# musaru/Fall_Multimodal

Measured on AMD Instinct MI355X. Metric: clips/sec (fwd+bwd) 3-stream Fall3, B=256, 1/2/4/8 GPUs; top-1 acc parity, higher is better.
Workload: dtype bf16x3; 1 GPU; fall3_3stream_coco_mmpose_V18_S6_B256_per_gpu; global_batch=256, seq_len=30, parallelism=dp1, joints=18, imu_axes=6, classes=11, hip_graph=False, ranks=1

## Files before the change

### fall_multimodal_amd/_lib.py

```python
from __future__ import annotations

import ctypes
import os

import torch

HERE = os.path.dirname(os.path.abspath(__file__))
LIB_PATH = os.environ.get("F3_LIB") or os.path.join(HERE, "libfall3.so")

EXPORTS = (
    "f3_net_create", "f3_net_destroy", "f3_net_num_entries", "f3_net_entry", "f3_net_param_count",
    "f3_net_buffer_count", "f3_net_counter_count", "f3_net_workspace_bytes", "f3_net_forward",
    "f3_net_loss", "f3_net_backward", "f3_rmsprop_step", "f3_conv_forward", "f3_status_string",
    "f3_net_debug_tensor", "f3_conv_backward_data", "f3_conv_backward_weight", "f3_conv_wgrad_packed", "f3_split_x3cat",
    "f3_conv_forward_x3cat", "f3_conv_backward_data_x3cat", "f3_conv_backward_weight_x3cat", "f3_conv_step_x3cat", "f3_graph_mix_forward",
    "f3_graph_mix_backward", "f3_graph_mix_forward_ex", "f3_graph_mix_backward_ex", "f3_gcn_dgrad_mix_x3",
    "f3_net_backward_phase",
    "f3_net_grad_split", "f3_net_wait_phase1", "f3_net_backward_rmsprop", "f3_net_fused_rmsprop", "f3_net_precision", "f3_net_status",
    "f3_targcn_create", "f3_targcn_destroy", "f3_targcn_num_entries", "f3_targcn_entry", "f3_targcn_param_count",
    "f3_targcn_buffer_count", "f3_targcn_workspace_bytes", "f3_targcn_forward", "f3_targcn_backward", "f3_targcn_stage_times", "f3_targcn_status", "f3_net_sensor_times", "f3_soft_ce",
    "f3_sktr_create", "f3_sktr_destroy", "f3_sktr_num_entries", "f3_sktr_entry", "f3_sktr_param_count",
    "f3_sktr_buffer_count", "f3_sktr_counter_count", "f3_sktr_workspace_bytes", "f3_sktr_forward", "f3_sktr_backward",
    "f3_musa_create", "f3_musa_destroy", "f3_musa_num_entries", "f3_musa_entry", "f3_musa_param_count",
    "f3_musa_buffer_count", "f3_musa_counter_count", "f3_musa_workspace_bytes", "f3_musa_forward", "f3_musa_backward",
    "f3_musa_guards",
    "f3_dwconv_t_forward", "f3_pointwise_conv", "f3_rgb_scratch_floats", "f3_rgb_forward", "f3_rgb_backward",
    "f3_optim_scalars_bytes", "f3_optim_step", "f3_optim_step_ranges", "f3_net_backward_optim", "f3_net_entry_nograd",
)

F3_OK, F3_EINVAL, F3_EBATCH, F3_EHIP, F3_ESTATE, F3_EDEVICE = 0, 1001, 1002, 1003, 1004, 1005
ENTRY_PARAM, ENTRY_BUFFER, ENTRY_COUNTER = 0, 1, 2
OPT_RMSPROP, OPT_SGD, OPT_ADAM, OPT_ADAMW = 0, 1, 2, 3
OPT_MAX_SKIP = 4


class F3OptimConfig(ctypes.Structure):
    _fields_ = ([("kind", ctypes.c_int), ("nesterov", ctypes.c_int)]
                + [(n, ctypes.c_double) for n in ("lr", "alpha", "eps", "momentum", "beta1", "beta2", "weight_decay",
                                                  "max_norm", "grad_scale")]
                + [("nskip", ctypes.c_int), ("skip_lo", ctypes.c_int64 * OPT_MAX_SKIP),
                   ("skip_len", ctypes.c_int64 * OPT_MAX_SKIP)])


class F3TargcnConfig(ctypes.Structure):
    _fields_ = [(n, ctypes.c_int) for n in ("num_node", "num_class", "precision")]


class F3MusaConfig(ctypes.Structure):
    _fields_ = [(n, ctypes.c_int) for n in ("num_point", "frames", "num_class", "precision")]


class F3SktrConfig(ctypes.Structure):
    _fields_ = [(n, ctypes.c_int) for n in ("num_joint", "frames", "persons", "num_class", "precision")]


class F3Config(ctypes.Structure):
    _fields_ = [(n, ctypes.c_int) for n in (
        "model", "num_node", "num_partition", "num_class", "in_channels", "sensor", "sensor_dim",
        "sensor_classes", "softmax_output", "naming", "frames", "sensor_frames", "precision")]


_lib = None


def lib():
    global _lib
    if _lib is not None:
        return _lib
    if not os.path.exists(LIB_PATH):
        raise RuntimeError(f"fall3: {LIB_PATH} is not built (run `make` or __graft_entry__.build())")
    L = ctypes.CDLL(LIB_PATH)
    P, I, I64, F = ctypes.c_void_p, ctypes.c_int, ctypes.c_int64, ctypes.c_float
    sig = {
        "f3_net_create": (I, [ctypes.POINTER(F3Config), ctypes.POINTER(P)]),
        "f3_net_destroy": (None, [P]),
        "f3_net_num_entries": (I, [P]),
        "f3_net_entry": (I, [P, I, ctypes.POINTER(ctypes.c_char_p), ctypes.POINTER(I), ctypes.POINTER(I),
                             ctypes.POINTER(I64), ctypes.POINTER(I64)]),
        "f3_net_param_count": (I64, [P]),
        "f3_net_buffer_count": (I64, [P]),
        "f3_net_counter_count": (I64, [P]),
        "f3_net_workspace_bytes": (I64, [P, I]),
        "f3_net_forward": (I, [P, I, I, P, P, P, P, P, P, P, P]),
        "f3_net_loss": (I, [P, I, P, P, P, P, P]),
        "f3_net_backward": (I, [P, I, P, P, P, P, P]),
        "f3_net_backward_phase": (I, [P, I, P, P, P, P, I, P]),
        "f3_net_grad_split": (I64, [P]),
        "f3_net_wait_phase1": (I, [P, P]),
        "f3_net_backward_rmsprop": (I, [P, I, P, P, P, P, P, F, F, F, P]),
        "f3_net_fused_rmsprop": (I, [P]),
        "f3_net_precision": (I, [P]),
        "f3_net_status": (I, [P, I]),
        "f3_rmsprop_step": (I, [P, P, P, I64, F, F, F, F, P]),
        "f3_optim_scalars_bytes": (I64, []),
        "f3_optim_step": (I, [ctypes.POINTER(F3OptimConfig), P, P, P, P, I64, P, P]),
        "f3_optim_step_ranges": (I, [ctypes.POINTER(F3OptimConfig), P, P, P, P, I, ctypes.POINTER(I64),
                                     ctypes.POINTER(I64), P, P]),
        "f3_net_backward_optim": (I, [P, I, P, P, P, P, P, P, P, ctypes.POINTER(F3OptimConfig), P]),
        "f3_net_entry_nograd": (I, [P, I]),
        "f3_conv_forward": (I, [P, P, P, P, P, I, I, I, I, I, I, I, I, I, P]),
        "f3_status_string": (ctypes.c_char_p, [I]),
        "f3_net_debug_tensor": (P, [P, I, P, I, I, ctypes.c_char_p]),
        "f3_conv_backward_data": (I, [P, P, P, P, I, I, I, I, I, I, I, I, I, P]),
        "f3_conv_backward_weight": (I, [P, P, P, P, I, I, I, I, I, I, I, I, I, P]),
        "f3_conv_wgrad_packed": (I, [P, P, P, ctypes.c_longlong, I, I, I, I, I, I, I, I, P]),
        "f3_split_x3cat": (I, [P, P, ctypes.c_int64, I, P]),
        "f3_conv_forward_x3cat": (I, [P, P, P, P, P, I, I, I, I, I, I, I, I, P]),
        "f3_conv_backward_data_x3cat": (I, [P, P, P, P, I, I, I, I, I, I, I, I, P]),
        "f3_conv_backward_weight_x3cat": (I, [P, P, P, P, I, I, I, I, I, I, I, I, P]),
        "f3_conv_step_x3cat": (I, [I, P, P, P, P, P, P, P, P, P, P, F, P, P, I, I, I, I, I, P]),
        "f3_graph_mix_forward": (I, [P, P, P, I, I, I, I, P]),
        "f3_graph_mix_backward": (I, [P, P, P, P, P, I, I, I, I, P]),
        "f3_graph_mix_forward_ex": (I, [P, P, P, I, I, I, I, I, P]),
        "f3_graph_mix_backward_ex": (I, [P, P, P, P, P, I, I, I, I, I, P]),
        "f3_gcn_dgrad_mix_x3": (I, [P, P, P, P, P, P, P, I, I, I, I, I, I, I, P]),
        "f3_targcn_create": (I, [ctypes.POINTER(F3TargcnConfig), ctypes.POINTER(P)]),
        "f3_targcn_destroy": (None, [P]),
        "f3_targcn_num_entries": (I, [P]),
        "f3_targcn_entry": (I, [P, I, ctypes.POINTER(ctypes.c_char_p), ctypes.POINTER(I), ctypes.POINTER(I),
                                ctypes.POINTER(I64), ctypes.POINTER(I64)]),
        "f3_targcn_param_count": (I64, [P]),
        "f3_targcn_buffer_count": (I64, [P]),
        "f3_targcn_workspace_bytes": (I64, [P, I]),
        "f3_targcn_stage_times": (I, [P, I, P]),
        "f3_targcn_status": (I, [P, I]),
        "f3_net_sensor_times": (I, [P, I, P]),
        "f3_targcn_forward": (I, [P, I, P, P, P, P, P, P]),
        "f3_targcn_backward": (I, [P, I, P, P, P, P, P, P]),
        "f3_soft_ce": (I, [P, P, I, I, P, P, P]),
        "f3_sktr_create": (I, [ctypes.POINTER(F3SktrConfig), ctypes.POINTER(P)]),
        "f3_sktr_destroy": (None, [P]),
        "f3_sktr_num_entries": (I, [P]),
        "f3_sktr_entry": (I, [P, I, ctypes.POINTER(ctypes.c_char_p), ctypes.POINTER(I), ctypes.POINTER(I),
                              ctypes.POINTER(I64), ctypes.POINTER(I64)]),
        "f3_sktr_param_count": (I64, [P]),
        "f3_sktr_buffer_count": (I64, [P]),
        "f3_sktr_counter_count": (I64, [P]),
        "f3_sktr_workspace_bytes": (I64, [P, I]),
        "f3_sktr_forward": (I, [P, I, I, P, P, P, P, P, P, P, ctypes.c_uint, F, P]),
        "f3_sktr_backward": (I, [P, I, P, P, P, P, P, P]),
        "f3_musa_create": (I, [ctypes.POINTER(F3MusaConfig), ctypes.POINTER(P)]),
        "f3_musa_destroy": (None, [P]),
        "f3_musa_num_entries": (I, [P]),
        "f3_musa_entry": (I, [P, I, ctypes.POINTER(ctypes.c_char_p), ctypes.POINTER(I), ctypes.POINTER(I),
                              ctypes.POINTER(I64), ctypes.POINTER(I64)]),
        "f3_musa_param_count": (I64, [P]),
        "f3_musa_buffer_count": (I64, [P]),
        "f3_musa_counter_count": (I64, [P]),
        "f3_musa_workspace_bytes": (I64, [P, I]),
        "f3_musa_guards": (I, [P, I, ctypes.POINTER(I64), I]),
        "f3_musa_forward": (I, [P, I, I, P, P, P, P, P, P, ctypes.c_uint, I, P]),
        "f3_musa_backward": (I, [P, I, P, P, P, P, P, P]),
        "f3_dwconv_t_forward": (I, [P, P, P, P, P, I, I, I, I, I, I, I, P]),
        "f3_pointwise_conv": (I, [P, P, P, P, I, P, P, I, I, I, I, I, I, I, I, I, P]),
        "f3_rgb_scratch_floats": (ctypes.c_longlong, [I, I]),
        "f3_rgb_forward": (I, [P, P, P, P, I, I, P]),
        "f3_rgb_backward": (I, [P, P, P, P, P, P, P, ctypes.c_longlong, I, I, P]),
    }
    for name, (res, args) in sig.items():
        fn = getattr(L, name)
        fn.restype = res
        fn.argtypes = args
    _lib = L
    return L


def check(status: int, what: str):
    if status == F3_OK:
# ... 19 lines not shown
```

### fall_multimodal_amd/csrc/layers.h

```cpp
#pragma once
#include "common.h"

namespace f3 {

enum : int { PREP_MUL = 0, PREP_PACK_CONV, PREP_PACK_CONV_T, PREP_PACK_GCN, PREP_PACK_GCN_T, PREP_GCN_BIAS, PREP_COPY,
              PREP_UNPACK_CONV };

struct PrepJob {
  int type, n;
  float* dst;
  const float* s0;
  const float* s1;
  const float* s2;
  int d0, d1, d2;
  int bf16;
};

struct DataBnArgs {
  int N, T, V, C, motion;
  const float* skel;
  float* out;
  int act16;
  BnRef bn;
  double* st_sum;
  double* st_sq;
  const float* dout;
  float* dgamma;
  float* dbeta;
  float* part;
};

struct MixArgs {
  int K, V, Cin, frames;
  const float* A;
  const float* x;
  int x16;
  float* z;
  float* dx;
  float* dA;
  int accumulate;
  float* part;
  unsigned short* zb;
  const unsigned short* dzb;
  int no_colsum;
  int x3;
  unsigned short* z3;
};
constexpr int kMixParts = 1024;

struct GcnDgradMixArgs {
  int frames, K, V, Cin, C;
  const unsigned short* dg;
  const unsigned short* w;
  const float* A;
  const float* x;
  float* dx;
  float* dA;
  int accumulate;
  float* part;
  int no_colsum;
  int max_workgroups;
};

struct Gcn0Args {
  int frames, K, V, Ci;
  const float* A;
  const unsigned short* x;
  const unsigned short* w;
  const float* beff;
  unsigned short* z;
  unsigned short* g;
  double* st_sum;
  double* st_sq;
  const unsigned short* dg;
  float* dx;
  int accumulate;
  float* part_dA;
  float* part_dW;
  int f32;
};

struct GcnBiasBwdArgs {
  int K, V, C;
  const float* Aeff;
  const float* A;
  const float* G;
  const float* bias;
  float* db;
  const float* dAeff;
  float* dE;
};

enum : int { RES_NONE = 0, RES_ID = 1, RES_CONV = 2 };

constexpr int kCaMaxRowsPerThread = 4;

struct BlockArgs {
  int N, TV, C, chunks, res_kind;
  int act16;
  float inv_tv;
  BnRef bn2, bnr;
  const float* h;
  const float* r;
  const float* x;
  const float* att;
  float* out;
  float* pool;
  unsigned short* outb;
  const float* dout;
  const float* dout_nc;
  float* P1;
  float* P2;
  float* Q2;
  double* bnr_bsum;
// ... 61 lines not shown
  const float* Q2;
  double* bnr_bsum;
  double* bnr_bsq;
  float* dq2;
  float* dbn;
  float* dq1;
  float* e;
  double* bn2_bsum;
  double* bn2_bsq;
  float* g_bnca_gamma;
  float* g_bnca_beta;
  float* g_b1;
  float* g_W1;
  float* g_W2;
  float* g_b2;
  float* wpart;
  const float* bpart;
  int bchunks;
};


struct BnRunJob {
  const double* sum;
  const double* sumsq;
  double count;
  int C;
  float* rmean;
  float* rvar;
  long long* nbt;
};

constexpr int kMaxPrepJobs = 56;
struct PrepTable {
  int n;
  PrepJob jobs[kMaxPrepJobs];
};
constexpr int kMaxBnJobs = 56;
struct BnRunTable {
  int n;
  BnRunJob jobs[kMaxBnJobs];
};

}

int f3_prep(const f3::PrepTable& t, hipStream_t s);
int f3_databn_fwd(const f3::DataBnArgs* a, hipStream_t s);
int f3_databn_bwd(const f3::DataBnArgs* a, hipStream_t s);
int f3_mix_fwd(const f3::MixArgs* a, hipStream_t s);
int f3_mix_bwd(const f3::MixArgs* a, hipStream_t s);
int f3_mix_bwd_parts(const f3::MixArgs* a);
bool f3_gcn_dgrad_mix_ok(int K, int V, int Cin, int C);
int f3_gcn_dgrad_mix(const f3::GcnDgradMixArgs* a, hipStream_t s);
int f3_gcn_dgrad_mix_parts(const f3::GcnDgradMixArgs* a);
bool f3_mix_lds_ok(int K, int V, int Cin);
bool f3_mix_x3_ok(int K, int V, int Cin);
int f3_split_x3(const float* x, unsigned short* out, long long rows, int C, hipStream_t s);
int f3_gcn_bias_bwd(const f3::GcnBiasBwdArgs* a, hipStream_t s);
bool f3_gcn0_ok(int K, int V, int Ci, int C);
int f3_gcn0_fwd(const f3::Gcn0Args* a, hipStream_t s);
int f3_gcn0_bwd(const f3::Gcn0Args* a, hipStream_t s);
int f3_gcn0_bwd_parts(const f3::Gcn0Args* a);
int f3_databn_bwd2(const f3::DataBnArgs* a, hipStream_t s);
int f3_block_out(f3::BlockArgs a, hipStream_t s);
int f3_block_bwd_reduce(f3::BlockArgs a, hipStream_t s);
int f3_block_bwd_apply(f3::BlockArgs a, hipStream_t s);
int f3_bn_bwd_apply(f3::BnBwdArgs a, hipStream_t s);
int f3_bn_bwd_parts(int N, int TV, int V);
int f3_block_chunks(int TV);
int f3_bnrelu_bf16(const f3::BnReluArgs* a, hipStream_t s);
constexpr int kColsumJobs = 10;
struct ColsumJob {
  const float* part;
  float* out;
  long long ld;
  int rows, cols;
};
int f3_colsum_multi(const ColsumJob* jobs, int n, hipStream_t s);
int f3_colsum(const float* part, int rows, int cols, float* out, hipStream_t s);
int f3_colsum_ld(const float* part, int rows, long long ld, int cols, float* out, hipStream_t s);
int f3_ca_fwd(const f3::CaArgs* a, hipStream_t s);
int f3_ca_bwd(const f3::CaArgs* a, hipStream_t s);
int f3_ca_bwd_weights(const f3::CaArgs* a, hipStream_t s, ColsumJob* defer = nullptr, int* ndefer = nullptr);
bool f3_ca_x_ok(int N, int C, int TV);
int f3_bn_running(const f3::BnRunTable& t, hipStream_t s);
```

### fall_multimodal_amd/csrc/net.cpp

```cpp
#include <hip/hip_runtime.h>

#include <algorithm>
#include <cstdio>
#include <functional>
#include <cstdlib>
#include <cstring>
#include <string>
#include <vector>

#include "common.h"
#include "status_ring.h"
#include "kernels.h"
#include "layers.h"
#include "sensor.h"
#include "fall3.h"

using namespace f3;

namespace {

struct Entry {
  std::string name;
  int kind;
  std::vector<int64_t> shape;
// ... 439 lines not shown
  float* G;
  float* opt_p = nullptr;
  float* opt_sq = nullptr;
  float lr = 0.f, alpha = 0.f, eps = 0.f;
  const OptLaunch* opt_gen = nullptr;
  const float* p(int i) const { return P + net.entries[i].offset; }
  float* g(int i) const { return G + net.entries[i].offset; }
  float* b(int i) const { return B + net.entries[i].offset; }
  long long* c(int i) const { return reinterpret_cast<long long*>(C + net.entries[i].offset); }
  BnRef ref(const BnIdx& bi, const BnWs& w, float count, int eval) const {
    BnRef r;
    r.sum = w.fsum;
    r.sumsq = w.fsq;
    r.gamma = p(bi.w);
    r.beta = p(bi.b);
    r.rmean = B ? b(bi.rm) : nullptr;
    r.rvar = B ? b(bi.rv) : nullptr;
    r.count = count;
    r.eval = eval;
    return r;
  }
};


ConvGeom geom(int M, int Nc, int Kc, int KT, int S, int P, int tr, int T_out, int T_in, int V, int lda, int ldo) {
  ConvGeom g;
  g.M = M; g.Nc = Nc; g.Kc = Kc; g.KT = KT; g.S = S; g.P = P; g.transposed = tr;
  g.T_out = T_out; g.T_in = T_in; g.V = V; g.lda = lda; g.ldo = ldo;
  return g;
}

void add_job(PrepTable& t, int type, int n, float* dst, const float* s0, const float* s1, const float* s2, int d0,
             int d1, int d2, int bf16 = 0) {
  PrepJob& j = t.jobs[t.n++];
  j.type = type; j.n = n; j.dst = dst; j.s0 = s0; j.s1 = s1; j.s2 = s2; j.d0 = d0; j.d1 = d1; j.d2 = d2;
  j.bf16 = bf16;
}

inline const unsigned short* bf(const float* p, int on) { return on ? reinterpret_cast<const unsigned short*>(p) : nullptr; }
inline int is_x3(const f3_net& n) { return n.cfg.precision == F3_PRECISION_BF16X3; }
inline int side_pct(bool split, int l) { return split && l >= 2 ? 75 : 0; }
constexpr int x3code() { return 4; }
inline int x3mul(int code) { return code == 4 ? 2 : 1; }
inline void x3_gemm(ConvGemmArgs& a, int C) {
  a.x3n = 1;
  a.g.lda = 2 * C;
}

inline bool gcn_dgrad_fused() {
  static const bool on = !getenv("F3_GCN_DGRAD_FUSED") || atoi(getenv("F3_GCN_DGRAD_FUSED")) != 0;
  return on;
}

inline int wcode(const f3_net& n) { return n.cfg.precision == F3_PRECISION_BF16 ? 1 : is_x3(n) ? 2 : 0; }
inline unsigned short* bfa(float* p, int on) { return on ? reinterpret_cast<unsigned short*>(p) : nullptr; }

void add_bnrun(BnRunTable& t, const Ptrs& q, const BnIdx& bi, const double* sum, const double* sq, double count) {
  BnRunJob& j = t.jobs[t.n++];
  j.sum = sum; j.sumsq = sq; j.count = count; j.C = bi.C;
  j.rmean = q.b(bi.rm); j.rvar = q.b(bi.rv); j.nbt = q.c(bi.nbt);
}

int stream_forward_layer(const f3_net& net, int si, int N, int train, const Ptrs& q, Ws& w, BnRunTable& run,
                         hipStream_t s, int l);

int stream_forward(const f3_net& net, int si, int N, int train, const Ptrs& q, Ws& w, const float* skel,
                   BnRunTable& run, hipStream_t s, int stage) {
  if (stage >= 0) return stream_forward_layer(net, si, N, train, q, w, run, s, stage);
  const StreamIdx& S = net.st[si];
  StreamWs& W = w.st[si];
  const int K = net.K, V = net.V, eval = !train;
  const int hb = net.cfg.precision == F3_PRECISION_BF16;
  const int wc = wcode(net);
  PrepTable pt;
  pt.n = 0;
  add_job(pt, PREP_COPY, K * V * V, W.A, q.b(S.A), nullptr, nullptr, 0, 0, 0);
  for (int l = 0; l < 7; ++l) {
    const LayerIdx& L = S.L[l];
    LayerWs& X = W.L[l];
    const int C = L.cout, Ci = L.cin;
    add_job(pt, PREP_MUL, K * V * V, X.aeff, q.b(S.A), q.p(L.edge), nullptr, 0, 0, 0);
    add_job(pt, PREP_GCN_BIAS, V * C, X.beff, q.b(S.A), q.p(L.edge), q.p(L.gcn_b), C, V, K);
    const bool l0f = wc == 2 && f3_gcn0_ok(K, V, Ci, C);
    const int xc = wc == 2 ? x3code() : wc;
    const int gc = wc == 2 && f3_mix_x3_ok(K, V, Ci) ? xc : (l0f ? 0 : wc);
    add_job(pt, PREP_PACK_GCN, C * K * Ci * x3mul(gc), X.gw, q.p(L.gcn_w), nullptr, nullptr, C, Ci, K, gc);
    add_job(pt, PREP_PACK_CONV, C * 9 * C * x3mul(xc), X.tw, q.p(L.tcn_w), nullptr, nullptr, C, C, 9, xc);
    if (train) {
      add_job(pt, PREP_PACK_GCN_T, C * K * Ci * x3mul(gc), X.gwT, q.p(L.gcn_w), nullptr, nullptr, C, Ci, K, gc);
      add_job(pt, PREP_PACK_CONV_T, C * 9 * C * x3mul(xc), X.twT, q.p(L.tcn_w), nullptr, nullptr, C, C, 9, xc);
    }
    if (L.res == RES_CONV) {
      add_job(pt, PREP_PACK_CONV, C * Ci * x3mul(xc), X.rw, q.p(L.res_w), nullptr, nullptr, C, Ci, 1, xc);
      if (train) add_job(pt, PREP_PACK_CONV_T, C * Ci * x3mul(xc), X.rwT, q.p(L.res_w), nullptr, nullptr, C, Ci, 1, xc);
    }
  }
  F3_TRY(f3_prep(pt, s));
  DataBnArgs d;
  std::memset(&d, 0, sizeof(d));
  d.N = N; d.T = S.T; d.V = V; d.C = S.cin; d.motion = S.motion; d.skel = skel; d.out = W.x0;
  d.bn = q.ref(S.dbn, W.dbn, (float)(N * S.T), eval);
  d.st_sum = W.dbn.fsum; d.st_sq = W.dbn.fsq;
  d.act16 = hb;
  F3_TRY(f3_databn_fwd(&d, s));
  if (train) add_bnrun(run, q, S.dbn, W.dbn.fsum, W.dbn.fsq, (double)N * S.T);
  return F3_OK;
}

int stream_forward_layer(const f3_net& net, int si, int N, int train, const Ptrs& q, Ws& w, BnRunTable& run,
                         hipStream_t s, int l) {
  const StreamIdx& S = net.st[si];
  StreamWs& W = w.st[si];
  const int K = net.K, V = net.V, eval = !train;
  const int hb = net.cfg.precision == F3_PRECISION_BF16;
  const int x3 = is_x3(net), wq = hb || x3;
  {
    const LayerIdx& L = S.L[l];
    LayerWs& X = W.L[l];
    const int C = L.cout, Ci = L.cin, Ti = L.T_in, To = L.T_out;
    const int Mi = N * Ti * V, Mo = N * To * V;
    const BnRef bn1 = q.ref(L.bn1, X.bn1, (float)Mi, eval);
    const BnRef bn2 = q.ref(L.bn2, X.bn2, (float)Mo, eval);
    BnRef bnr;
    std::memset(&bnr, 0, sizeof(bnr));
    if (L.res == RES_CONV) bnr = q.ref(L.bnr, X.bnr, (float)Mo, eval);
    if ((hb || x3) && f3_gcn0_ok(K, V, Ci, C)) {
      Gcn0Args g0;
      std::memset(&g0, 0, sizeof(g0));
      g0.frames = N * Ti; g0.K = K; g0.V = V; g0.Ci = Ci; g0.A = X.aeff;
      g0.x = reinterpret_cast<const unsigned short*>(X.x); g0.w = bf(X.gw, 1); g0.beff = X.beff;
      g0.z = bfa(X.z, 1); g0.g = bfa(X.g, 1); g0.st_sum = X.bn1.fsum; g0.st_sq = X.bn1.fsq;
      g0.f32 = x3;
      F3_TRY(f3_gcn0_fwd(&g0, s));
    } else {
      MixArgs mx;
      std::memset(&mx, 0, sizeof(mx));
      mx.K = K; mx.V = V; mx.Cin = Ci; mx.frames = N * Ti; mx.A = X.aeff; mx.x = X.x; mx.z = X.z;
      mx.zb = bfa(X.z, hb); mx.x16 = hb; mx.x3 = x3;
      const bool gcat = x3 && f3_mix_x3_ok(K, V, Ci);
      mx.z3 = bfa(X.z, gcat);
      F3_TRY(f3_mix_fwd(&mx, s));
      ConvGemmArgs ga;
      std::memset(&ga, 0, sizeof(ga));
      ga.g = geom(Mi, C, K * Ci, 1, 1, 0, 0, Ti, Ti, V, K * Ci, C);
      ga.in = hb ? nullptr : X.z; ga.inb = bfa(X.z, hb); ga.zero = w.zero;
      ga.w = X.gw; ga.wb = bf(X.gw, wq); ga.out = X.g; ga.outb = bfa(X.g, hb); ga.x3 = x3;
      ga.bias = X.beff; ga.st_sum = X.bn1.fsum; ga.st_sq = X.bn1.fsq;
      if (gcat) {
        ga.x3 = 0; ga.in = nullptr; ga.inb = bfa(X.z, 1);
        x3_gemm(ga, K * Ci);
      }
      F3_TRY(f3_conv_gemm(&ga, 0, EPI_BIASV | EPI_STATS, s));
    }
    if (L.res == RES_CONV) {
      ConvGemmArgs ra;
      std::memset(&ra, 0, sizeof(ra));
      ra.g = geom(Mo, C, Ci, 1, L.stride, 0, 0, To, Ti, V, Ci, C);
      ra.in = hb ? nullptr : X.x; ra.inb = hb ? X.xb : nullptr; ra.zero = w.zero;
      if (hb && !X.xb) return F3_ESTATE;
      ra.w = X.rw; ra.wb = bf(X.rw, wq); ra.out = X.r; ra.outb = bfa(X.r, hb); ra.x3 = x3;
      ra.bias = q.p(L.res_b); ra.st_sum = X.bnr.fsum; ra.st_sq = X.bnr.fsq;
      if (x3) {
        if (!X.xb) return F3_ESTATE;
        ra.x3 = 0; ra.in = nullptr; ra.inb = X.xb;
        x3_gemm(ra, Ci);
      }
      F3_TRY(f3_conv_gemm(&ra, 0, EPI_BIAS | EPI_STATS, s));
    }
    ConvGemmArgs ta;
    std::memset(&ta, 0, sizeof(ta));
    ta.g = geom(Mo, C, C, 9, L.stride, 4, 0, To, Ti, V, C, C);
    ta.w = X.tw; ta.wb = bf(X.tw, wq); ta.out = X.h; ta.outb = bfa(X.h, hb); ta.bias = q.p(L.tcn_b);
    ta.st_sum = X.bn2.fsum; ta.st_sq = X.bn2.fsq; ta.gap = X.gap;
    if (hb || x3) {
      BnReluArgs br;
      std::memset(&br, 0, sizeof(br));
      br.M = Mi; br.C = C; br.bn = bn1; br.g = X.g; br.u = X.u; br.g16 = hb; br.x3 = x3;
      F3_TRY(f3_bnrelu_bf16(&br, s));
      if (x3) x3_gemm(ta, C);
      ta.inb = X.u; ta.zero = w.zero;
      F3_TRY(f3_conv_gemm(&ta, 0, EPI_BIAS | EPI_STATS | EPI_GAP, s));
    } else {
      ta.in = X.g; ta.pro_bn = bn1;
      F3_TRY(f3_conv_gemm(&ta, 1, EPI_BIAS | EPI_STATS | EPI_GAP, s));
    }
    CaArgs ca;
// ... 1175 lines not shown
  m.x = static_cast<const float*>(x); m.x16 = flags & F3_MIX_X_BF16; m.x3 = (flags & F3_MIX_X3) != 0;
  m.z = static_cast<float*>(z);
  if (flags & F3_MIX_Z_BF16) m.zb = static_cast<unsigned short*>(z);
  if (flags & F3_MIX_Z3) m.z3 = static_cast<unsigned short*>(z);
  return f3_mix_fwd(&m, (hipStream_t)stream);
}

int f3_graph_mix_backward_ex(const float* A_eff, const void* x, const void* dz, float* dx, float* dA, int frames, int K,
                             int V, int Cin, int flags, void* stream) {
  if (!A_eff || !x || !dz || !dx || !dA || frames < 0 || (flags & ~5) || ((flags & F3_MIX_X3) && (flags & 1)))
    return F3_EINVAL;
  hipStream_t s = (hipStream_t)stream;
  if (hipMemsetAsync(dA, 0, sizeof(float) * K * V * V, s) != hipSuccess) return F3_EHIP;
  MixArgs m;
  std::memset(&m, 0, sizeof(m));
  m.K = K; m.V = V; m.Cin = Cin; m.frames = frames; m.A = A_eff; m.x = static_cast<const float*>(x);
  m.dx = dx; m.dA = dA; m.accumulate = 0; m.x3 = (flags & F3_MIX_X3) != 0;
  if (flags & F3_MIX_X_BF16) {
    m.x16 = 1;
    m.dzb = static_cast<const unsigned short*>(dz);
  } else {
    m.z = const_cast<float*>(static_cast<const float*>(dz));
  }
  static float* part = nullptr;
  if (!part && hipMalloc(&part, sizeof(float) * kMixParts * 1024) != hipSuccess) return F3_EHIP;
  m.part = part;
  return f3_mix_bwd(&m, s);
}

int f3_gcn_dgrad_mix_x3(const void* dg3, const float* w, void* wpack, const float* A_eff, const float* x, float* dx,
                        float* dA, int frames, int K, int V, int Cin, int C, int accumulate, int max_workgroups,
                        void* stream) {
  hipStream_t s = (hipStream_t)stream;
  if (!dg3 || !wpack || !A_eff || !x || !dx || !dA || frames < 0 || max_workgroups < 0) return F3_EINVAL;
  if (!f3_gcn_dgrad_mix_ok(K, V, Cin, C) || K * V * V > 1024) return F3_EINVAL;
  if (w) {
    PrepTable t;
    t.n = 0;
    add_job(t, PREP_PACK_CONV_T, C * K * Cin * x3mul(x3code()), static_cast<float*>(wpack), w, nullptr, nullptr, C,
            K * Cin, 1, x3code());
    F3_TRY(f3_prep(t, s));
  }
  if (hipMemsetAsync(dA, 0, sizeof(float) * K * V * V, s) != hipSuccess) return F3_EHIP;
  static float* part = nullptr;
  if (!part && hipMalloc(&part, sizeof(float) * kMixParts * 1024) != hipSuccess) return F3_EHIP;
  GcnDgradMixArgs a;
  std::memset(&a, 0, sizeof(a));
  a.frames = frames; a.K = K; a.V = V; a.Cin = Cin; a.C = C; a.dg = static_cast<const unsigned short*>(dg3);
  a.w = static_cast<const unsigned short*>(wpack); a.A = A_eff; a.x = x; a.dx = dx; a.dA = dA;
  a.accumulate = accumulate != 0; a.part = part; a.max_workgroups = max_workgroups;
  return f3_gcn_dgrad_mix(&a, s);
}

void* f3_net_debug_tensor(f3_net* net, int batch, void* workspace, int stream, int layer, const char* what) {
  if (!net || stream < 0 || stream >= net->nstreams || layer < 0 || layer > 6) return nullptr;
  Ws w = plan(*net, batch, (char*)workspace);
  StreamWs& W = w.st[stream];
  LayerWs& X = W.L[layer];
  const std::string k(what);
  if (k == "x") return (void*)X.x;
  if (k == "z") return X.z;
  if (k == "g") return X.g;
  if (k == "h") return X.h;
  if (k == "r") return X.r;
  if (k == "out") return X.out;
  if (k == "att") return X.att;
  if (k == "dh") return X.dh;
  if (k == "u") return X.u;
  if (k == "dv") return W.dv;
  if (k == "dg") return X.dg;
  if (k == "dZ") return W.dZ;
  if (k == "dres") return X.dres;
  if (k == "dx0") return W.dx[0];
  if (k == "dx1") return W.dx[1];
  if (k == "bn1_fsum") return X.bn1.fsum;
  if (k == "bn1_fsq") return X.bn1.fsq;
  if (k == "bn1_bsum") return X.bn1.bsum;
  if (k == "bn1_bsq") return X.bn1.bsq;
  if (k == "twT") return X.twT;
  if (k == "P1") return X.P1;
  if (k == "P2") return X.P2;
  if (k == "e") return X.e;
  if (k == "gap") return X.gap;
  if (k == "q1") return X.q1;
  if (k == "hid") return X.hid;
  if (k == "dq1") return X.dq1;
  if (k == "dq2") return X.dq2;
  if (k == "dbn") return X.dbn;
  if (k == "bn2_fsum") return X.bn2.fsum;
  if (k == "bn2_fsq") return X.bn2.fsq;
  if (k == "bn2_bsum") return X.bn2.bsum;
  if (k == "bn2_bsq") return X.bn2.bsq;
  if (k == "ca_fsum") return X.bnca.fsum;
  if (k == "ca_fsq") return X.bnca.fsq;
  if (k == "dpool") return W.dpool;
  if (k == "pool") return W.pool;
  return nullptr;
}

const char* f3_status_string(int st) {
  switch (st) {
    case F3_OK: return "ok";
    case F3_EINVAL: return "invalid argument or unsupported shape";
    case F3_EBATCH: return "Expected more than 1 value per channel when training";
    case F3_EHIP: return "HIP launch error";
    case F3_ESTATE: return "backward without a training forward";
// ... 7 lines not shown
```

### include/fall3.h

```cpp
#ifndef FALL3_H
#define FALL3_H
#include <stdint.h>

#ifdef __cplusplus
extern "C" {
#endif

#define F3_OK 0
#define F3_EINVAL 1001
#define F3_EBATCH 1002
#define F3_EHIP 1003
#define F3_ESTATE 1004
#define F3_EDEVICE 1005

enum { F3_MODEL_TWO_STGCAN_BILSTM = 0, F3_MODEL_TWO_STGCAN = 1, F3_MODEL_STGCN = 2, F3_MODEL_BILSTM = 3 };
enum { F3_SENSOR_NONE = 0, F3_SENSOR_BILSTM = 1, F3_SENSOR_CNN_BILSTM = 2 };
enum { F3_NAMING_PACKAGE = 0, F3_NAMING_NOTEBOOK = 1 };
enum { F3_PRECISION_FP32 = 0,
       F3_PRECISION_BF16 = 1,
       F3_PRECISION_BF16_FP32IN = 2,
       F3_PRECISION_BF16X3 = 4  };
enum { F3_ENTRY_PARAM = 0, F3_ENTRY_BUFFER = 1, F3_ENTRY_COUNTER = 2 };

typedef struct f3_config {
// ... 74 lines not shown
int f3_optim_step_ranges(const f3_optim_config* cfg, float* params, float* state0, float* state1,
                         const float* grads, int nranges, const int64_t* lo, const int64_t* len, void* scalars,
                         void* stream);
int f3_net_backward_optim(f3_net* net, int batch, float* params, const float* dout, float* grads, float* state0,
                          float* state1, void* scalars, void* workspace, const f3_optim_config* cfg, void* stream);
int f3_net_entry_nograd(const f3_net* net, int i);

enum { F3_CONV_BF16_OUT = 3 };
int f3_conv_forward(const void* x, const float* w, const float* bias, float* out, float* wpack, int N, int T_in,
                    int V, int Cin, int Cout, int KT, int stride, int pad, int precision, void* stream);

int f3_conv_backward_data(const void* dy, const float* w, float* dx, float* wpack, int N, int T_in, int V, int Cin,
                          int Cout, int KT, int stride, int pad, int precision, void* stream);
int f3_conv_backward_weight(const void* dy, const void* x, float* dw, float* db, int N, int T_in, int V, int Cin,
                            int Cout, int KT, int stride, int pad, int precision, void* stream);
int f3_conv_wgrad_packed(const void* dy, const void* x, float* slab, long long slab_floats, int N, int T_in, int V,
                         int Cin, int Cout, int KT, int stride, int pad, void* stream);

#define F3_STEP_GCN_FWD 0
#define F3_STEP_TCN_DGRAD 1
int f3_split_x3cat(const float* x, void* out, int64_t rows, int C, void* stream);
int f3_conv_forward_x3cat(const void* x3, const float* w, const float* bias, float* out, void* wpack, int N, int T_in,
                          int V, int Cin, int Cout, int KT, int stride, int pad, void* stream);
int f3_conv_backward_data_x3cat(const void* dy3, const float* w, float* dx, void* wpack, int N, int T_in, int V,
                                int Cin, int Cout, int KT, int stride, int pad, void* stream);
int f3_conv_backward_weight_x3cat(const void* dy3, const void* x3, float* dw, float* db, int N, int T_in, int V,
                                  int Cin, int Cout, int KT, int stride, int pad, void* stream);
int f3_conv_step_x3cat(int kind, const void* in3, const float* w, void* wpack, float* out, const float* bias_v,
                       const float* g, const float* gamma, const float* beta, const double* bn_sum,
                       const double* bn_sq, float bn_count, double* st_sum, double* st_sq, int N, int T, int V,
                       int Cin, int Cout, void* stream);

int f3_pointwise_conv(const void* x, const void* wpack, const float* bias, void* out, int out_bf16, double* st_sum,
                      double* st_sq, int N, int T_in, int T_out, int V, int Cin, int Cout, int stride, int transposed,
                      int epi, void* stream);

long long f3_rgb_scratch_floats(int B, int T);
int f3_rgb_forward(const void* frames, const void* wpack, const float* bias, float* feat, int B, int T, void* stream);
int f3_rgb_backward(const void* frames, const void* wpack, const float* bias, const float* dfeat, float* dw, float* db,
                    float* scratch, long long scratch_floats, int B, int T, void* stream);

int f3_graph_mix_forward(const float* A_eff, const float* x, float* z, int frames, int K, int V, int Cin,
                         void* stream);
int f3_graph_mix_backward(const float* A_eff, const float* x, const float* dz, float* dx, float* dA, int frames, int K,
                          int V, int Cin, void* stream);
enum { F3_MIX_X_BF16 = 1, F3_MIX_Z_BF16 = 2, F3_MIX_X3 = 4, F3_MIX_Z3 = 8 };
int f3_graph_mix_forward_ex(const float* A_eff, const void* x, void* z, int frames, int K, int V, int Cin, int flags,
                            void* stream);
int f3_graph_mix_backward_ex(const float* A_eff, const void* x, const void* dz, float* dx, float* dA, int frames, int K,
                             int V, int Cin, int flags, void* stream);
int f3_gcn_dgrad_mix_x3(const void* dg3, const float* w, void* wpack, const float* A_eff, const float* x, float* dx,
                        float* dA, int frames, int K, int V, int Cin, int C, int accumulate, int max_workgroups,
                        void* stream);

const char* f3_status_string(int status);

typedef struct f3_targcn_config {
  int num_node;
  int num_class;
  int precision;
} f3_targcn_config;

typedef struct f3_targcn f3_targcn;

int f3_targcn_create(const f3_targcn_config* cfg, f3_targcn** out);
void f3_targcn_destroy(f3_targcn* net);
int f3_targcn_num_entries(const f3_targcn* net);
int f3_targcn_entry(const f3_targcn* net, int i, const char** name, int* kind, int* ndim, int64_t* shape8,
                    int64_t* offset);
int64_t f3_targcn_param_count(const f3_targcn* net);
int64_t f3_targcn_buffer_count(const f3_targcn* net);
int64_t f3_targcn_workspace_bytes(const f3_targcn* net, int batch);
int f3_targcn_forward(f3_targcn* net, int batch, const float* params, const float* buffers, const float* source,
                      float* out, void* workspace, void* stream);
int f3_targcn_backward(f3_targcn* net, int batch, const float* params, const float* buffers, const float* dout,
                       float* grads, void* workspace, void* stream);
int f3_targcn_stage_times(f3_targcn* net, int enable, float* ms);
int f3_targcn_status(f3_targcn* net, int wait);
int f3_soft_ce(const float* out, const float* label, int N, int C, float* loss, float* dout, void* stream);

typedef struct f3_musa_config {
  int num_point;
  int frames;
  int num_class;
  int precision;
} f3_musa_config;

typedef struct f3_musa f3_musa;

int f3_musa_create(const f3_musa_config* cfg, f3_musa** out);
void f3_musa_destroy(f3_musa* net);
int f3_musa_num_entries(const f3_musa* net);
int f3_musa_entry(const f3_musa* net, int i, const char** name, int* kind, int* ndim, int64_t* shape8,
                  int64_t* offset);
int64_t f3_musa_param_count(const f3_musa* net);
int64_t f3_musa_buffer_count(const f3_musa* net);
int64_t f3_musa_counter_count(const f3_musa* net);
int64_t f3_musa_workspace_bytes(const f3_musa* net, int batch);
int f3_musa_forward(f3_musa* net, int batch, int training, const float* params, float* buffers, int64_t* counters,
                    const float* x, float* out, void* workspace, unsigned seed, int dropout, void* stream);
int f3_musa_backward(f3_musa* net, int batch, const float* params, const float* buffers, const float* dout,
                     float* grads, void* workspace, void* stream);
int f3_musa_guards(const f3_musa* net, int batch, int64_t* offsets, int max);
int f3_dwconv_t_forward(const float* x, const float* w, const float* b, float* y, double* sums, int N, int T_in,
                        int V, int C, int K, int S, int P, void* stream);

// ... 32 lines not shown
```

Measured before the change: 33100 clips/s.

## Fuse GCN forward graph mix, x3 pointwise GEMM, bias and BN stats into one kernel

Result: faster. 33660 clips/s (median of 6 runs) (+1.7%).

```diff
diff --git a/fall_multimodal_amd/_lib.py b/fall_multimodal_amd/_lib.py
--- a/fall_multimodal_amd/_lib.py
+++ b/fall_multimodal_amd/_lib.py
@@ -15,6 +15,7 @@
     "f3_net_debug_tensor", "f3_conv_backward_data", "f3_conv_backward_weight", "f3_conv_wgrad_packed", "f3_split_x3cat",
     "f3_conv_forward_x3cat", "f3_conv_backward_data_x3cat", "f3_conv_backward_weight_x3cat", "f3_conv_step_x3cat", "f3_graph_mix_forward",
     "f3_graph_mix_backward", "f3_graph_mix_forward_ex", "f3_graph_mix_backward_ex", "f3_gcn_dgrad_mix_x3",
+    "f3_gcn_fwd_mix_x3",
     "f3_net_backward_phase",
     "f3_net_grad_split", "f3_net_wait_phase1", "f3_net_backward_rmsprop", "f3_net_fused_rmsprop", "f3_net_precision", "f3_net_status",
     "f3_targcn_create", "f3_targcn_destroy", "f3_targcn_num_entries", "f3_targcn_entry", "f3_targcn_param_count",
@@ -114,6 +115,7 @@
         "f3_graph_mix_forward_ex": (I, [P, P, P, I, I, I, I, I, P]),
         "f3_graph_mix_backward_ex": (I, [P, P, P, P, P, I, I, I, I, I, P]),
         "f3_gcn_dgrad_mix_x3": (I, [P, P, P, P, P, P, P, I, I, I, I, I, I, I, P]),
+        "f3_gcn_fwd_mix_x3": (I, [P, P, P, P, P, P, P, P, P, I, I, I, I, I, P]),
         "f3_targcn_create": (I, [ctypes.POINTER(F3TargcnConfig), ctypes.POINTER(P)]),
         "f3_targcn_destroy": (None, [P]),
         "f3_targcn_num_entries": (I, [P]),
diff --git a/fall_multimodal_amd/csrc/gcn_fwd.hip b/fall_multimodal_amd/csrc/gcn_fwd.hip
--- /dev/null
+++ b/fall_multimodal_amd/csrc/gcn_fwd.hip
@@ -0,0 +1,325 @@
+#include "igemm.h"
+#include "layers.h"
+
+#include <algorithm>
+#include <cstdlib>
+#include <type_traits>
+
+namespace f3 {
+
+constexpr int GF_THREADS = 512;
+constexpr int GF_VMAX = 18, GF_K = 3, GF_CIN = 64, GF_KC = GF_K * GF_CIN;
+constexpr int GF_BM = 32, GF_KS = 2 * GF_KC / 32;
+constexpr int GF_XD = 7, GF_NXB = GF_XD + 1;
+constexpr int GF_RING = GF_BM * GF_NXB;
+constexpr int GF_ZP = GF_BM * 4 * GF_KC / 16 / GF_THREADS;
+
+template <int WN>
+struct GfLds {
+  static constexpr int NT = 64 * WN;
+  static constexpr int ABUF = GF_BM * GF_KC * 2 * 2;
+  static constexpr int OTS = NT + 4;
+  static constexpr int X_OFF = 2 * ABUF;
+  static constexpr int OT_OFF = X_OFF + GF_RING * GF_CIN * 4;
+  static constexpr int BV_OFF = OT_OFF + GF_BM * OTS * 4;
+  static constexpr int RED_OFF = BV_OFF + GF_VMAX * NT * 4;
+  static constexpr int BYTES = RED_OFF + 2 * 2 * NT * 4;
+  static constexpr int PIECES = GF_BM * NT * 4 / 16 / GF_THREADS;
+};
+
+typedef __bf16 gf_bf16x4 __attribute__((ext_vector_type(4)));
+typedef unsigned gf_u32x4 __attribute__((ext_vector_type(4)));
+
+F3_DEV void gf_a_split(float t, __bf16& hi, __bf16& lo) {
+  const float h = __uint_as_float(__float_as_uint(t) & 0xffff0000u);
+  hi = __builtin_bit_cast(__bf16, (unsigned short)(__float_as_uint(h) >> 16));
+  lo = (__bf16)(t - h);
+}
+
+F3_DEV float gf_atil(const float* A, int K, int V, int wk, int v) {
+  if (wk >= K * V || v >= V) return 0.f;
+  const int w = wk / K, k = wk - w * K;
+  return A[(k * V + v) * V + w];
+}
+
+F3_DEV f32x4 gf_mfma_x3m(bf16x8 ah, bf16x8 al, bf16x8 bh, bf16x8 bl, f32x4 c) {
+  c = mfma_bf16x(al, bh, c);
+  c = mfma_bf16x(ah, bl, c);
+  return mfma_bf16x(ah, bh, c);
+}
+
+template <int WN>
+__global__ __launch_bounds__(GF_THREADS) void gcn_fwd_mix_x3_kernel(GcnFwdMixArgs a, int per_wg) {
+  using L = GfLds<WN>;
+  constexpr int NT = L::NT, OTS = L::OTS, KS = GF_KS, K = GF_K, CIN = GF_CIN, PIECES = L::PIECES;
+  constexpr int OPS = 1 + GF_ZP + PIECES;
+  constexpr int NSTEADY = GF_ZP + OPS * (GF_XD - 2);
+  static_assert(L::BYTES <= 160 * 1024 && NSTEADY < 64 && GF_ZP * GF_THREADS * 16 == L::ABUF, "gcn_fwd LDS / vmcnt");
+  static_assert((GF_RING & (GF_RING - 1)) == 0 && PIECES >= 1, "ring");
+  extern __shared__ __attribute__((aligned(16))) char gf_smem[];
+  char* img = gf_smem + L::OT_OFF;
+  float* bv = reinterpret_cast<float*>(gf_smem + L::BV_OFF);
+  float* red = reinterpret_cast<float*>(gf_smem + L::RED_OFF);
+  const int tid = threadIdx.x, lane = tid & 63;
+  const int wave = __builtin_amdgcn_readfirstlane(tid >> 6);
+  const int wm = wave & 1, wj = wave >> 1;
+  const int mt = wave & 3, nh = wave >> 2;
+  const int fr = lane & 15, fg = lane >> 4;
+  const int V = a.V, KV = K * V, M = a.frames * V;
+  const int ntiles = (M + GF_BM - 1) / GF_BM;
+  const int range = xcd_remap(blockIdx.x, gridDim.x);
+  const int tile0 = range * per_wg, tile1 = min(ntiles, tile0 + per_wg);
+  if (tile0 >= tile1) return;
+
+  const int rbase = (tile0 - 1) * GF_BM;
+  const int mend = min(M, (tile1 + 1) * GF_BM);
+  char* xring = gf_smem + L::X_OFF;
+  auto load_block = [&](int b) {
+    const int m = b * GF_BM + wave * 4 + (lane >> 4);
+    const void* src = (m >= 0 && m < mend) ? (const void*)(a.x + (size_t)m * CIN + (lane & 15) * 4) : (const void*)a.zero;
+    char* dst = xring + (((b * GF_BM - rbase) & (GF_RING - 1)) + wave * 4) * (CIN * 4);
+    __builtin_amdgcn_global_load_lds(src, (lds_void_t*)dst, 16, 0, 0);
+  };
+#pragma unroll
+  for (int i = 0; i < (GF_VMAX * NT * 4 + 8191) / 8192; ++i) {
+    const int o = (wave + 8 * i) * 1024;
+    if (o < V * NT * 4) {
+      const void* src = o + lane * 16 < V * NT * 4 ? (const void*)(reinterpret_cast<const char*>(a.bias) + o + lane * 16)
+                                                   : (const void*)a.zero;
+      __builtin_amdgcn_global_load_lds(src, (lds_void_t*)(gf_smem + L::BV_OFF + o), 16, 0, 0);
+    }
+  }
+#pragma unroll
+  for (int i = 0; i < GF_NXB; ++i) load_block(tile0 - 1 + i);
+
+  bf16x8 wf[WN][KS];
+#pragma unroll
+  for (int y = 0; y < WN; ++y) {
+    const unsigned short* wr = a.w + (size_t)(wj * 16 * WN + y * 16 + fr) * (2 * GF_KC) + fg * 8;
+#pragma unroll
+    for (int s = 0; s < KS; ++s) wf[y][s] = *reinterpret_cast<const bf16x8*>(wr + s * 32);
+  }
+  bf16x8 bhi[2], blo[2];
+#pragma unroll
+  for (int q = 0; q < 2; ++q)
+#pragma unroll
+    for (int e = 0; e < 8; ++e) {
+      __bf16 h, l;
+      gf_a_split(gf_atil(a.A, K, V, 16 * (2 * nh + q) + fr, 8 * fg + e), h, l);
+      bhi[q][e] = h;
+      blo[q][e] = l;
+    }
+  float ssum[WN], ssq[WN];
+#pragma unroll
+  for (int y = 0; y < WN; ++y) ssum[y] = ssq[y] = 0.f;
+  asm volatile("s_waitcnt vmcnt(0) lgkmcnt(0)" ::: "memory");
+#pragma unroll
+  for (int y = 0; y < WN; ++y)
+#pragma unroll
+    for (int s = 0; s < KS; ++s) asm volatile("" ::"v"(wf[y][s]));
+#pragma unroll
+  for (int q = 0; q < 2; ++q) asm volatile("" ::"v"(bhi[q]), "v"(blo[q]));
+  __builtin_amdgcn_s_barrier();
+  const unsigned x_lds = (unsigned)(size_t)(lds_void_t*)xring;
+  const unsigned a_lds = (unsigned)(size_t)(lds_void_t*)gf_smem;
+  const unsigned img_lds = (unsigned)(size_t)(lds_void_t*)img;
+
+  auto mix_frame = [&](int f) {
+    const int rel0 = f * V - rbase;
+    float xv[8];
+#pragma unroll
+    for (int e = 0; e < 8; ++e) {
+      const int v = min(8 * fg + e, V - 1);
+      const unsigned ad = x_lds + (unsigned)(((rel0 + v) & (GF_RING - 1)) * (CIN * 4) + (16 * mt + fr) * 4);
+      asm volatile("ds_read_b32 %0, %1" : "=v"(xv[e]) : "v"(ad));
+    }
+    asm volatile("s_waitcnt lgkmcnt(0)"
+                 : "+v"(xv[0]), "+v"(xv[1]), "+v"(xv[2]), "+v"(xv[3]), "+v"(xv[4]), "+v"(xv[5]), "+v"(xv[6]), "+v"(xv[7])
+                 :
+                 : "memory");
+    bf16x8 xah, xal;
+#pragma unroll
+    for (int e = 0; e < 8; ++e) {
+      const float x = 8 * fg + e < V ? xv[e] : 0.f;
+      const __bf16 h = (__bf16)x;
+      xah[e] = h;
+      xal[e] = (__bf16)(x - (float)h);
+    }
+#pragma unroll
+    for (int q = 0; q < 2; ++q) {
+      const int wk = 16 * (2 * nh + q) + fr;
+      const f32x4 acc = gf_mfma_x3m(xah, xal, bhi[q], blo[q], f32x4{0.f, 0.f, 0.f, 0.f});
+      const int w = wk / K, k = wk - w * K;
+      const int m = f * V + w, tt = m >> 5, r = m & 31;
+      gf_bf16x4 h, l;
+#pragma unroll
+      for (int e = 0; e < 4; ++e) {
+        h[e] = (__bf16)acc[e];
+        l[e] = (__bf16)(acc[e] - (float)h[e]);
+      }
+      if (wk < KV && tt >= tile0 && tt < tile1) {
+        char* row = gf_smem + ((tt - tile0) & 1) * L::ABUF + ((2 * k + (mt >> 1)) * GF_BM + r) * 128 + (fg & 1) * 8;
+        const int p = 2 * (mt & 1) + (fg >> 1);
+        *reinterpret_cast<gf_bf16x4*>(row + swz(r, p) * 16) = h;
+        *reinterpret_cast<gf_bf16x4*>(row + swz(r, 4 + p) * 16) = l;
+      }
+    }
+  };
+
+  constexpr int CPR = NT * 4 / 16;
+  auto store_g = [&](int tile, auto full) {
+    gf_u32x4 v[PIECES];
+#pragma unroll
+    for (int i = 0; i < PIECES; ++i) {
+      const int q = tid + i * GF_THREADS, rl = q / CPR, c = q - rl * CPR;
+      asm volatile("ds_read_b128 %0, %1" : "=v"(v[i]) : "v"(img_lds + (unsigned)(rl * OTS * 4 + c * 16)));
+    }
+    if constexpr (PIECES == 1) asm volatile("s_waitcnt lgkmcnt(0)" : "+v"(v[0])::"memory");
+    else asm volatile("s_waitcnt lgkmcnt(0)" : "+v"(v[0]), "+v"(v[PIECES - 1])::"memory");
+#pragma unroll
+    for (int i = 0; i < PIECES; ++i) {
+      const int q = tid + i * GF_THREADS, rl = q / CPR, c = q - rl * CPR;
+      const int m = tile * GF_BM + rl;
+      if (!decltype(full)::value && m >= M) continue;
+      *reinterpret_cast<gf_u32x4*>(reinterpret_cast<char*>(a.g + (size_t)m * NT) + c * 16) = v[i];
+    }
+  };
+  static_assert(GF_ZP == 3, "store_z waits for three reads");
+  auto store_z = [&](int tile, int buf, auto full) {
+    gf_u32x4 v[GF_ZP];
+#pragma unroll
+    for (int i = 0; i < GF_ZP; ++i) {
+      const int q = tid + i * GF_THREADS, rl = q / 48, j = q - rl * 48;
+      const int lo = j >= 24, jj = j - 24 * lo, b = jj >> 2, p = (jj & 3) + 4 * lo;
+      asm volatile("ds_read_b128 %0, %1"
+                   : "=v"(v[i])
+                   : "v"(a_lds + (unsigned)(buf * L::ABUF + (b * GF_BM + rl) * 128 + swz(rl, p) * 16)));
+    }
+    asm volatile("s_waitcnt lgkmcnt(0)" : "+v"(v[0]), "+v"(v[1]), "+v"(v[2])::"memory");
+#pragma unroll
+    for (int i = 0; i < GF_ZP; ++i) {
+      const int q = tid + i * GF_THREADS, rl = q / 48, j = q - rl * 48;
+      const int m = tile * GF_BM + rl;
+      if (!decltype(full)::value && m >= M) continue;
+      *reinterpret_cast<gf_u32x4*>(reinterpret_cast<char*>(a.z3) + (size_t)m * (4 * GF_KC) + j * 16) = v[i];
+    }
+  };
+
+  int fnext = (tile0 * GF_BM) / V;
+  auto body = [&](int tile, auto first, auto full) {
+    const int it = tile - tile0, buf = it & 1;
+    if constexpr (!decltype(first)::value) store_g(tile - 1, std::true_type{});
+    const int flast = (min(tile * GF_BM + GF_BM, M) - 1) / V;
+    for (; fnext <= flast; ++fnext) mix_frame(fnext);
+    asm volatile("s_waitcnt lgkmcnt(0)" ::: "memory");
+    __builtin_amdgcn_s_barrier();
+    load_block(tile + GF_XD);
+    store_z(tile, buf, full);
+    const char* A = gf_smem + buf * L::ABUF;
+    f32x4 acc[WN];
+#pragma unroll
+    for (int y = 0; y < WN; ++y) acc[y] = f32x4{0.f, 0.f, 0.f, 0.f};
+#pragma unroll
+    for (int b = 0; b < KS / 2; ++b) {
+      const int r = wm * 16 + fr;
+      const bf16x8 fah = *reinterpret_cast<const bf16x8*>(A + (b * GF_BM + r) * 128 + swz(r, fg) * 16);
+      const bf16x8 fal = *reinterpret_cast<const bf16x8*>(A + (b * GF_BM + r) * 128 + swz(r, 4 + fg) * 16);
+#pragma unroll
+      for (int y = 0; y < WN; ++y) {
+        acc[y] = mfma_bf16x(fah, wf[y][2 * b], acc[y]);
+        acc[y] = mfma_bf16x(fal, wf[y][2 * b], acc[y]);
+        acc[y] = mfma_bf16x(fah, wf[y][2 * b + 1], acc[y]);
+      }
+    }
+    asm volatile("s_waitcnt lgkmcnt(0)" ::: "memory");
+    __builtin_amdgcn_s_barrier();
+#pragma unroll
+    for (int r = 0; r < 4; ++r) {
+      const int rl = wm * 16 + fg * 4 + r, m = tile * GF_BM + rl;
+      const bool ok = m < M;
+      const int vj = (ok ? m : 0) % V;
+#pragma unroll
+      for (int y = 0; y < WN; ++y) {
+        const int jl = wj * 16 * WN + y * 16 + fr;
+        float v = acc[y][r];
+        v += bv[vj * NT + jl];
+        if (!ok) v = 0.f;
+        ssum[y] += v;
+        ssq[y] += v * v;
+        reinterpret_cast<float*>(img)[rl * OTS + jl] = v;
+      }
+    }
+    asm volatile("s_waitcnt vmcnt(%0) lgkmcnt(0)" ::"n"(NSTEADY) : "memory");
+    __builtin_amdgcn_s_barrier();
+  };
+  const bool ragged = tile1 == ntiles && M % GF_BM != 0;
+  const int tfull = ragged ? tile1 - 1 : tile1;
+  if (tile0 < tfull) {
+    body(tile0, std::true_type{}, std::true_type{});
+    for (int tile = tile0 + 1; tile < tfull; ++tile) body(tile, std::false_type{}, std::true_type{});
+    if (ragged) body(tile1 - 1, std::false_type{}, std::false_type{});
+  } else {
+    body(tile0, std::true_type{}, std::false_type{});
+  }
+  store_g(tile1 - 1, std::false_type{});
+#pragma unroll
+  for (int y = 0; y < WN; ++y) {
+    ssum[y] += __shfl_xor(ssum[y], 16, 64);
+    ssum[y] += __shfl_xor(ssum[y], 32, 64);
+    ssq[y] += __shfl_xor(ssq[y], 16, 64);
+    ssq[y] += __shfl_xor(ssq[y], 32, 64);
+  }
+  if (fg == 0) {
+#pragma unroll
+    for (int y = 0; y < WN; ++y) {
+      red[(wm * 2 + 0) * NT + wj * 16 * WN + y * 16 + fr] = ssum[y];
+      red[(wm * 2 + 1) * NT + wj * 16 * WN + y * 16 + fr] = ssq[y];
+    }
+  }
+  __syncthreads();
+  for (int t = tid; t < 2 * NT; t += GF_THREADS) {
+    const int q = t / NT, j = t - q * NT;
+    const float s = red[(0 * 2 + q) * NT + j] + red[(1 * 2 + q) * NT + j];
+    atomic_add_d((q == 0 ? a.st_sum : a.st_sq) + j, (double)s);
+  }
+  asm volatile("s_waitcnt vmcnt(0)" ::: "memory");
+}
+
+}
+
+using namespace f3;
+
+bool f3_gcn_fwd_mix_ok(int K, int V, int Cin, int C) {
+  return K == GF_K && Cin == GF_CIN && V >= 1 && V <= GF_VMAX && (C == 64 || C == 128);
+}
+
+template <int WN>
+static int gf_launch(const GcnFwdMixArgs& a, int grid, int per_wg, hipStream_t s) {
+  constexpr int lds = GfLds<WN>::BYTES;
+  F3_LDS_LIMIT((gcn_fwd_mix_x3_kernel<WN>), lds);
+  hipLaunchKernelGGL((gcn_fwd_mix_x3_kernel<WN>), dim3(grid), dim3(GF_THREADS), lds, s, a, per_wg);
+  F3_LAUNCH_CHECK();
+  return F3_OK;
+}
+
+int f3_gcn_fwd_mix(const GcnFwdMixArgs* args, hipStream_t s) {
+  const GcnFwdMixArgs& a = *args;
+  if (!f3_gcn_fwd_mix_ok(a.K, a.V, a.Cin, a.C) || a.frames < 0) return F3_EINVAL;
+  if (!a.A || !a.x || !a.z3 || !a.w || !a.bias || !a.g || !a.st_sum || !a.st_sq || !a.zero) return F3_EINVAL;
+  if ((long long)a.frames * a.V >= (1ll << 31) - 64 * GF_BM) return F3_EINVAL;
+  if ((reinterpret_cast<uintptr_t>(a.x) | reinterpret_cast<uintptr_t>(a.bias) | reinterpret_cast<uintptr_t>(a.z3) |
+       reinterpret_cast<uintptr_t>(a.g) | reinterpret_cast<uintptr_t>(a.w)) & 15)
+    return F3_EINVAL;
+  if (a.frames == 0) return F3_OK;
+  static int cus = [] {
+    int dev = 0, n = 256;
+    if (hipGetDevice(&dev) == hipSuccess) (void)hipDeviceGetAttribute(&n, hipDeviceAttributeMultiprocessorCount, dev);
+    (void)hipGetLastError();
+    return n;
+  }();
+  const int ntiles = (a.frames * a.V + GF_BM - 1) / GF_BM;
+  const int nr0 = std::max(1, cus);
+  const int per_wg = (ntiles + nr0 - 1) / nr0;
+  const int grid = (ntiles + per_wg - 1) / per_wg;
+  return a.C == 64 ? gf_launch<1>(a, grid, per_wg, s) : gf_launch<2>(a, grid, per_wg, s);
+}
diff --git a/fall_multimodal_amd/csrc/layers.h b/fall_multimodal_amd/csrc/layers.h
--- a/fall_multimodal_amd/csrc/layers.h
+++ b/fall_multimodal_amd/csrc/layers.h
@@ -60,6 +60,19 @@
   float* part;
   int no_colsum;
   int max_workgroups;
+};
+
+struct GcnFwdMixArgs {
+  int frames, K, V, Cin, C;
+  const float* A;
+  const float* x;
+  unsigned short* z3;
+  const unsigned short* w;
+  const float* bias;
+  float* g;
+  double* st_sum;
+  double* st_sq;
+  const unsigned short* zero;
 };
 
 struct Gcn0Args {
@@ -227,6 +240,8 @@
 bool f3_gcn_dgrad_mix_ok(int K, int V, int Cin, int C);
 int f3_gcn_dgrad_mix(const f3::GcnDgradMixArgs* a, hipStream_t s);
 int f3_gcn_dgrad_mix_parts(const f3::GcnDgradMixArgs* a);
+bool f3_gcn_fwd_mix_ok(int K, int V, int Cin, int C);
+int f3_gcn_fwd_mix(const f3::GcnFwdMixArgs* a, hipStream_t s);
 bool f3_mix_lds_ok(int K, int V, int Cin);
 bool f3_mix_x3_ok(int K, int V, int Cin);
 int f3_split_x3(const float* x, unsigned short* out, long long rows, int C, hipStream_t s);
diff --git a/fall_multimodal_amd/csrc/net.cpp b/fall_multimodal_amd/csrc/net.cpp
--- a/fall_multimodal_amd/csrc/net.cpp
+++ b/fall_multimodal_amd/csrc/net.cpp
@@ -515,6 +515,11 @@
   return on;
 }
 
+inline bool gcn_fwd_fused() {
+  static const bool on = !getenv("F3_GCN_FWD_FUSED") || atoi(getenv("F3_GCN_FWD_FUSED")) != 0;
+  return on;
+}
+
 inline int wcode(const f3_net& n) { return n.cfg.precision == F3_PRECISION_BF16 ? 1 : is_x3(n) ? 2 : 0; }
 inline unsigned short* bfa(float* p, int on) { return on ? reinterpret_cast<unsigned short*>(p) : nullptr; }
 
@@ -595,6 +600,14 @@
       g0.z = bfa(X.z, 1); g0.g = bfa(X.g, 1); g0.st_sum = X.bn1.fsum; g0.st_sq = X.bn1.fsq;
       g0.f32 = x3;
       F3_TRY(f3_gcn0_fwd(&g0, s));
+    } else if (x3 && f3_mix_x3_ok(K, V, Ci) && Ci == 64 && K * Ci == 192 && V <= 18 && (C == 64 || C == 128) &&
+               gcn_fwd_fused() && f3_gcn_fwd_mix_ok(K, V, Ci, C)) {
+      GcnFwdMixArgs gf;
+      std::memset(&gf, 0, sizeof(gf));
+      gf.frames = N * Ti; gf.K = K; gf.V = V; gf.Cin = Ci; gf.C = C; gf.A = X.aeff; gf.x = X.x;
+      gf.z3 = bfa(X.z, 1); gf.w = bf(X.gw, 1); gf.bias = X.beff; gf.g = X.g;
+      gf.st_sum = X.bn1.fsum; gf.st_sq = X.bn1.fsq; gf.zero = w.zero;
+      F3_TRY(f3_gcn_fwd_mix(&gf, s));
     } else {
       MixArgs mx;
       std::memset(&mx, 0, sizeof(mx));
@@ -1876,6 +1889,27 @@
   return f3_gcn_dgrad_mix(&a, s);
 }
 
+int f3_gcn_fwd_mix_x3(const float* A_eff, const float* x, const float* w, void* wpack, const float* bias_v, void* z3,
+                      float* g, double* st_sum, double* st_sq, int frames, int K, int V, int Cin, int C,
+                      void* stream) {
+  hipStream_t s = (hipStream_t)stream;
+  if (!A_eff || !x || !wpack || !bias_v || !z3 || !g || !st_sum || !st_sq || frames < 0) return F3_EINVAL;
+  if (!f3_gcn_fwd_mix_ok(K, V, Cin, C)) return F3_EINVAL;
+  if (w) {
+    PrepTable t;
+    t.n = 0;
+    add_job(t, PREP_PACK_CONV, C * K * Cin * x3mul(x3code()), static_cast<float*>(wpack), w, nullptr, nullptr, C,
+            K * Cin, 1, x3code());
+    F3_TRY(f3_prep(t, s));
+  }
+  GcnFwdMixArgs a;
+  std::memset(&a, 0, sizeof(a));
+  a.frames = frames; a.K = K; a.V = V; a.Cin = Cin; a.C = C; a.A = A_eff; a.x = x;
+  a.z3 = static_cast<unsigned short*>(z3); a.w = static_cast<const unsigned short*>(wpack); a.bias = bias_v; a.g = g;
+  a.st_sum = st_sum; a.st_sq = st_sq; a.zero = test_zero_page();
+  return f3_gcn_fwd_mix(&a, s);
+}
+
 void* f3_net_debug_tensor(f3_net* net, int batch, void* workspace, int stream, int layer, const char* what) {
   if (!net || stream < 0 || stream >= net->nstreams || layer < 0 || layer > 6) return nullptr;
   Ws w = plan(*net, batch, (char*)workspace);
diff --git a/include/fall3.h b/include/fall3.h
--- a/include/fall3.h
+++ b/include/fall3.h
@@ -150,6 +150,9 @@
 int f3_gcn_dgrad_mix_x3(const void* dg3, const float* w, void* wpack, const float* A_eff, const float* x, float* dx,
                         float* dA, int frames, int K, int V, int Cin, int C, int accumulate, int max_workgroups,
                         void* stream);
+int f3_gcn_fwd_mix_x3(const float* A_eff, const float* x, const float* w, void* wpack, const float* bias_v, void* z3,
+                      float* g, double* st_sum, double* st_sq, int frames, int K, int V, int Cin, int C,
+                      void* stream);
 
 const char* f3_status_string(int status);
 
```
